# kiudee/bayes-skopt

Hardware: AMD Instinct MI355X
Metric: mcmc_lml_evals_per_s_n2048 (higher is better)
Workload: dtype f64

## Files before the change

bayes-skopt_amd/csrc/bgp_chol.hip:

```cpp
#include "bgp_common.h"
#include "bgp_device.h"

#include "bgp_gemm.h"

#include <cstdlib>
#include <vector>

#ifdef PF_TRACE
__device__ unsigned long long pf_trace[32];
__device__ unsigned long long pf_trace_w[8 * 32];
#define PF_T(i) do { if (threadIdx.x == 0 && blockIdx.x == 0) pf_trace[i] = wall_clock64(); } while (0)
#define PF_TW(i) do { if ((threadIdx.x & 63) == 0 && blockIdx.x == 0) pf_trace_w[(threadIdx.x >> 6) * 32 + (i)] = wall_clock64(); } while (0)
extern "C" int bgp_debug_potrf_trace(unsigned long long* out) {
  return hipMemcpyFromSymbol(out, HIP_SYMBOL(pf_trace), sizeof(pf_trace)) == hipSuccess ? 0 : 1;
}
extern "C" int bgp_debug_potrf_trace_w(unsigned long long* out) {
  return hipMemcpyFromSymbol(out, HIP_SYMBOL(pf_trace_w), sizeof(pf_trace_w)) == hipSuccess ? 0 : 1;
}
#else
#define PF_T(i)
#define PF_TW(i)
#endif
#include "bgp_pf.h"
#include "bgp_mcmc.h"

template <int GEN, int STAT, int FORM>
__global__ void __launch_bounds__(PF_THREADS) potrf_kernel(double* __restrict__ Kbuf, double* __restrict__ Wbuf,
                                                     double* __restrict__ yw, double* __restrict__ accb,
                                                     double* __restrict__ lml, int* __restrict__ status, int n,
                                                     int ld, size_t mstride, int ystride, int nblk, int k, PfGen gen) {
  const int b = blockIdx.x;
  if (!GEN && status[b] != 0) return;
  PfPre nopre;
  nopre.state = 0;
  (void)pf_block<GEN, STAT, FORM, 0>(b, Kbuf, Wbuf, yw, accb, lml, status, n, ld, mstride, ystride, nblk, k, gen, false, nullptr,
                                     PsArgs(), nopre);
}

template <int STAT, int FORM>
__global__ void __launch_bounds__(PF_THREADS) mcmc_small_kernel(McmcArgs a, int h, double* __restrict__ lml, int* __restrict__ status,
                                                               int n, PfGen gen) {
#pragma clang fp contract(off)
  __shared__ double sh_qv[64], sh_pt[64];
  __shared__ double sh_prior;
  __shared__ int sh_acc;
  const int i = blockIdx.x, tid = threadIdx.x, p = a.p;
  const int m = a.movers[(size_t)h * a.Ns + i], pr = a.partners[(size_t)h * a.Ns + i];
  if (tid < p) {
    const double z = a.zz[(size_t)h * a.Ns + i];
    const double s = a.coords[(size_t)m * p + tid], c = a.coords[(size_t)pr * p + tid];
    const double v = c - (c - s) * z;
    sh_qv[tid] = v;
    if (!(v > -INFINITY && v < INFINITY)) {
      a.info[0] = 1u;
      if (v != v) {
        if (a.info[3] == 0u) a.info[3] = (unsigned)h + 1u;
      } else if (a.info[2] == 0u) {
        a.info[2] = (unsigned)h + 1u;
      }
    }
    sh_pt[tid] = mcmc_prior(a.prior_kind[tid], a.prior_par + 5 * tid, v);
  }
  __syncthreads();
  if (tid == 0) {
    double lp = 0.0;
    for (int k = 0; k < p; k++) lp += sh_pt[k];
    sh_prior = lp;
  }
  if (tid < a.hp) a.dh[(size_t)i * a.hp + tid] = a.h_src[tid] >= 0 ? sh_qv[a.h_src[tid]] : a.h_fixed[tid];
  __syncthreads();
  PfPre nopre;
  nopre.state = 0;
  (void)pf_block<1, STAT, FORM, 0>(i, nullptr, nullptr, nullptr, nullptr, lml, status, n, 128, (size_t)0, 0, 1, 0, gen, false, nullptr,
                                   PsArgs(), nopre);
  __syncthreads();
  if (tid == 0) {
    double lp = sh_prior + lml[i];
    if (!(lp > -INFINITY && lp < INFINITY)) lp = -INFINITY;
    const bool acc = a.factors[(size_t)h * a.Ns + i] + lp - a.logp[m] > a.logu[(size_t)h * a.Ns + i];
    if (acc) {
      a.logp[m] = lp;
      a.nacc[m] += 1;
    }
    sh_acc = acc ? 1 : 0;
    a.lps[(size_t)(h >> 1) * a.W + m] = acc ? lp : a.logp[m];
  }
  __syncthreads();
  if (tid < p) {
    const double v = sh_acc ? sh_qv[tid] : a.coords[(size_t)m * p + tid];
    if (sh_acc) a.coords[(size_t)m * p + tid] = v;
    a.chain[((size_t)(h >> 1) * a.W + m) * p + tid] = v;
  }
}

int bgp_launch_mcmc_small(bgp_ctx* ctx, hipStream_t st, const McmcArgs& a, int h) {
  if (a.p > 64 || a.hp > 64) {
    bgp_set_error("bgp_launch_mcmc_small: more than 64 entries per walker");
    return BGP_ERR_INVALID;
  }
  PfGen g;
  g.X = ctx->dXeff;
  g.alpha = ctx->dalpha;
  g.H = ctx->dh;
  g.y = ctx->dy;
  g.d = ctx->d;
  KB_DISPATCH(ctx->ks.stationary, ctx->ks.form,
              hipLaunchKernelGGL((mcmc_small_kernel<S, F>), dim3(a.Ns), dim3(PF_THREADS), 0, st, a, h, ctx->dlml, ctx->dstatus, ctx->n, g));
  BGP_HIP(hipGetLastError());
  return BGP_OK;
}

__global__ void pivot_root_kernel(const double* __restrict__ x, double* __restrict__ s, double* __restrict__ iv, int n) {
  const int i = blockIdx.x * blockDim.x + threadIdx.x;
  if (i >= n) return;
  double a, b;
  pf_pivot_root(x[i], a, b);
  s[i] = a;
  iv[i] = b;
}
extern "C" int bgp_debug_pivot_root(int device, int n, const double* x, double* sqrt_out, double* rsqrt_out) {
  if (n <= 0 || !x || !sqrt_out || !rsqrt_out) {
    bgp_set_error("bgp_debug_pivot_root: bad argument");
    return BGP_ERR_INVALID;
  }
  BGP_HIP(hipSetDevice(device));
  double* d = nullptr;
  BGP_HIP(hipMalloc(&d, (size_t)3 * n * sizeof(double)));
  hipError_t e = hipMemcpy(d, x, (size_t)n * sizeof(double), hipMemcpyHostToDevice);
  if (e == hipSuccess) {
    hipLaunchKernelGGL(pivot_root_kernel, dim3((n + 255) / 256), dim3(256), 0, 0, d, d + n, d + 2 * (size_t)n, n);
    e = hipMemcpy(sqrt_out, d + n, (size_t)n * sizeof(double), hipMemcpyDeviceToHost);
  }
  if (e == hipSuccess) e = hipMemcpy(rsqrt_out, d + 2 * (size_t)n, (size_t)n * sizeof(double), hipMemcpyDeviceToHost);
  (void)hipFree(d);
  BGP_HIP(e);
  return BGP_OK;
}

int bgp_ps_total_tasks(int B, int nblk, int np, int gen);
void bgp_launch_ps(hipStream_t st, const PsArgs& a, int nwg);

extern "C" int bgp_debug_ps_trace(bgp_ctx* c, int* dims, unsigned long long* out, size_t cap) {
  if (!c || !dims) return BGP_ERR_INVALID;
  dims[0] = c->ps_trace_B;
  dims[1] = c->ps_trace_nblk;
  dims[2] = c->ps_trace_total;
  const size_t need = (size_t)c->ps_trace_B * c->ps_trace_nblk * 8 + (size_t)c->ps_trace_total * 8;
  if (!out || !c->ps_trace || need == 0) return BGP_OK;
  if (cap < need) return BGP_ERR_INVALID;
  BGP_HIP(hipSetDevice(c->device));
  BGP_HIP(hipMemcpy(out, c->ps_trace, need * sizeof(unsigned long long), hipMemcpyDeviceToHost));
  return BGP_OK;
}

int bgp_persist_fits(bgp_ctx* c, int B) {
  return B >= 1 && B <= 64 && c->nblk >= 2 && c->nblk <= 255 && c->ncu - B >= std::max(32, B);
}

int bgp_ps_ensure_flags(bgp_ctx* c, int B) {
  const size_t words = ps_flag_words(B, c->nblk);
  if (words > c->cap_psflags) {
    if (c->ps_flags) (void)hipFree(c->ps_flags);
    c->ps_flags = nullptr;
    c->cap_psflags = 0;
    BGP_HIP(hipMalloc(&c->ps_flags, (words + words / 2) * sizeof(unsigned)));
    c->cap_psflags = words + words / 2;
  }
  return BGP_OK;
}

int bgp_launch_cholesky_persist(bgp_ctx* c, int B, int build_gram) {
  const int nblk = c->nblk, ld = c->npad;
  if (!bgp_persist_fits(c, B)) {
    bgp_set_error("bgp_launch_cholesky_persist: B = %d, nblk = %d outside the persistent path's range", B, nblk);
    return BGP_ERR_INVALID;
  }
  const int ncu = c->ncu;
  if (!c->ps_herr) {
    BGP_HIP(hipHostMalloc((void**)&c->ps_herr, sizeof(unsigned), hipHostMallocDefault));
    *c->ps_herr = 0;
  }
  const size_t words = ps_flag_words(B, nblk);
  {
    const int rcf = bgp_ps_ensure_flags(c, B);
    if (rcf) return rcf;
  }
  if (!c->ps_resident) BGP_HIP(hipMemsetAsync(c->ps_flags, 0, words * sizeof(unsigned), c->stream));
  static unsigned long long limit = 0;
  if (!limit) {
    const char* e = getenv("BGP_PS_TIMEOUT_MS");
    limit = 100000ull * (unsigned long long)((e && atoi(e) > 0) ? atoi(e) : 500);
    const char* et = getenv("BGP_PS_TIMEOUT_TICKS");
    if (et && atoll(et) > 0) limit = (unsigned long long)atoll(et);
  }
  PsArgs a;
  a.K = c->dK;
  a.W = c->dW;
  a.yw = c->dyw;
  a.acc = c->dacc;
  a.lml = c->dlml;
  a.status = c->dstatus;
  a.flags = c->ps_flags;
  a.n = c->n;
  a.ld = ld;
  a.nblk = nblk;
  a.B = B;
  a.ystride = ld;
  a.mstride = (size_t)ld * ld;
  {
    static int want = -2;
    if (want == -2) {
      const char* e = getenv("BGP_PS_PAIR");
      want = e ? (atoi(e) != 0 ? 1 : 0) : -1;
    }
    a.Bpad = 8 * ((B + 7) / 8);
    const bool fits = nblk >= 3 && ncu - 2 * a.Bpad >= std::max(32, B);
    a.pair = (fits && (want == 1 || (want == -1 && bgp_pair_auto_rule(nblk, B)))) ? 1 : 0;
    a.nchain = a.pair ? 2 * a.Bpad : B;
    a.psplit = a.pair ? 4 : 1;
    a.dsplit = a.psplit == 4 ? 3 : 1;
    a.total = bgp_ps_total_tasks(B, nblk, a.psplit, 0);
    a.ncrit_stream = 3;
  }
  int tile_wgs = std::min(a.total, ncu - a.nchain);
  {
    const int auto_crit = nblk <= 10 ? ((a.pair || B > 32) ? std::min((a.psplit + 1 + a.dsplit + (a.psplit == 4 ? 4 : 0)) * B, tile_wgs / 2) : 0)
                                     : (a.pair && a.psplit == 4 ? std::min(B == 1 ? 48 : 96, tile_wgs / 2) : 0);
    a.ncrit = auto_crit;
    if (a.ncrit > tile_wgs - 1) a.ncrit = std::max(0, tile_wgs - 1);
  }
  a.gen = 0;
  if (build_gram) {
    static int want = -2;
    if (want == -2) {
      const char* e = getenv("BGP_PS_GEN");
      want = e ? (atoi(e) != 0 ? 1 : 0) : -1;
    }
    const bool can = !a.pair && a.ncrit == 0 && a.total > 0 && c->ks.stationary == BGP_MATERN52 && c->ks.form == BGP_FORM_PRODUCT;
    if (can && (want == 1 || (want == -1 && bgp_ps_gen_auto_rule(nblk, B)))) {
      a.gen = 1;
      a.total = bgp_ps_total_tasks(B, nblk, a.psplit, 1);
    } else {
      const int rck = bgp_launch_kbuild(c, B, 0, 0, 1);
      if (rck) return rck;
    }
  }
  a.d = c->d;
  a.X = c->dXeff;
  a.alpha = c->dalpha;
  a.H = c->dh;
  a.y = c->dy;
  tile_wgs = std::min(a.total, ncu - a.nchain);
  a.spin_limit = limit;
  a.trace = nullptr;
  {
    static int want = -1;
    if (want < 0) {
      const char* e = getenv("BGP_PS_TRACE");
      want = (e && atoi(e) != 0) ? 1 : 0;
    }
    if (want) {
      const size_t need = (size_t)B * nblk * 8 + (size_t)a.total * 8;
      if (need > c->cap_pstrace) {
        if (c->ps_trace) (void)hipFree(c->ps_trace);
        c->ps_trace = nullptr;
        c->cap_pstrace = 0;
        BGP_HIP(hipMalloc(&c->ps_trace, need * sizeof(unsigned long long)));
        c->cap_pstrace = need;
      }
      BGP_HIP(hipMemsetAsync(c->ps_trace, 0, need * sizeof(unsigned long long), c->stream));
      a.trace = c->ps_trace;
      c->ps_trace_B = B;
      c->ps_trace_nblk = nblk;
      c->ps_trace_total = a.total;
    }
  }
  bgp_launch_ps(c->stream, a, a.nchain + tile_wgs);
  if (!c->ps_resident)
    BGP_HIP(hipMemcpyAsync(c->ps_herr, c->ps_flags + PS_ERROR, sizeof(unsigned), hipMemcpyDeviceToHost, c->stream));
  BGP_HIP(hipGetLastError());
  return BGP_OK;
}

void bgp_launch_syrk4(hipStream_t st, int B8, double* dK, const int* dstatus, int ld, size_t mstride, int nblk, int kp,
                      int K, int jstart, int colmode, int B);
void bgp_launch_trsm4(hipStream_t st, int B, double* dK, double* dW, double* dyw, int* dstatus, int ld, size_t mstride,
                      int ystride, int nblk, int k, int augmented);

void bgp_launch_potrf(bgp_ctx* ctx, hipStream_t st, int B, double* dK, double* dW, double* dyw, double* dacc,
                      double* dlml, int* dstatus, int ld, size_t mstride, int ystride, int k) {
  hipLaunchKernelGGL((potrf_kernel<0, 0, 0>), dim3(B), dim3(PF_THREADS), 0, st, dK, dW, dyw, dacc, dlml, dstatus, ctx->n, ld,
                     mstride, ystride, ctx->nblk, k, PfGen());
}

int bgp_launch_lml_small(bgp_ctx* ctx, int off, int B, hipStream_t st) {
  PfGen g;
  g.X = ctx->dXeff;
  g.alpha = ctx->dalpha;
  g.H = ctx->dh + (size_t)off * (ctx->d + 2);
  g.y = ctx->dy;
  g.d = ctx->d;
  bgp_tbegin(ctx, 1, st);
  KB_DISPATCH(ctx->ks.stationary, ctx->ks.form,
              hipLaunchKernelGGL((potrf_kernel<1, S, F>), dim3(B), dim3(PF_THREADS), 0, st, (double*)nullptr,
                                 (double*)nullptr, (double*)nullptr, (double*)nullptr, ctx->dlml + off, ctx->dstatus + off,
                                 ctx->n, 128, (size_t)0, 0, 1, 0, g));
  bgp_tend(ctx, st);
  BGP_HIP(hipGetLastError());
  return BGP_OK;
}

void bgp_launch_syrk4_gen(hipStream_t st, int B8, double* dK, const int* dstatus, int ld, size_t mstride, int nblk, int kp,
                          int K, int jstart, int colmode, int B, const S4Gen& gen, int stationary, int form);

int bgp_launch_cholesky(bgp_ctx* ctx, int B, int augmented) {
  return bgp_launch_cholesky_slice(ctx, 0, B, ctx->stream, augmented);
}

int bgp_launch_cholesky_slice(bgp_ctx* ctx, int off, int B, hipStream_t st, int augmented, int gen) {
  const int nblk = ctx->nblk, npad = ctx->npad;
  const int ld = augmented ? 2 * npad : npad;
  const size_t mstride = (size_t)ld * ld;
  const int ystride = ld;
  const int B8 = 8 * ((B + 7) / 8);
  double* dK = ctx->dK + (size_t)off * mstride;
  double* dW = ctx->dW + (size_t)off * nblk * (128 * 128);
  double* dyw = ctx->dyw + (size_t)off * ystride;
  double* dacc = ctx->dacc + (size_t)off * 4;
  double* dlml = ctx->dlml + off;
  int* dstatus = ctx->dstatus + off;
  if (!augmented) {
    const int P = ctx->panels_auto ? (nblk >= 12 ? 4 : 2) : ctx->panels;
    S4Gen ga{};
    if (gen) {
      const int rcg = bgp_lml_gen_args(ctx, off, &ga);
      if (rcg) return rcg;
      ctx->gen_batches++;
    }
    int k = 0;
// ... 53 lines not shown
```

bayes-skopt_amd/csrc/bgp_pf.h:

```cpp
#pragma once
#include "bgp_common.h"
#include "bgp_device.h"
#include "bgp_gemm.h"

#ifndef PF_T
#define PF_T(i)
#endif
#ifndef PF_TW
#define PF_TW(i)
#endif
#define PF_LD 130
#define PF_MLD 18

template <int C>
static __device__ __forceinline__ double bc16(double v) {
  return __builtin_amdgcn_update_dpp(v, v, 0x150 + C, 0xF, 0xF, false);
}

#define PF_FMAC_BCAST(D, SRC, S1, C)                                                                  \
  asm volatile("v_fmac_f64_dpp %0, %1, %2 row_newbcast:%3 row_mask:0xf bank_mask:0xf" : "+v"(D) : "v"(SRC), "v"(S1), "n"(C))

template <int J, int C>
static __device__ __forceinline__ void micro_cols(double (&a)[16], double (&macc)[16], double naj, double mj) {
  if constexpr (C < 16) {
    PF_FMAC_BCAST(a[C], a[J], naj, C);
    PF_FMAC_BCAST(macc[C], a[J], mj, C);
    micro_cols<J, C + 1>(a, macc, naj, mj);
  }
}

static __device__ __forceinline__ void pf_pivot_root(double x, double& dj, double& inv) {
  const double y0 = __builtin_amdgcn_rsq(x);
  const double g = x * y0, h = 0.5 * y0;
  const double r = fma(-g, h, 0.5);
  const double g1 = fma(g, r, g);
  const double y1 = fma(y0, r, y0);
  const double hy = 0.5 * y1;
  const double d = fma(-g1, g1, x);
  dj = fma(d, hy, g1);
  const double e = fma(-dj, y1, 1.0);
  inv = fma(y1, e, y1);
}

template <int J>
static __device__ __forceinline__ void micro_chol_inv(double (&a)[16], double (&macc)[16], double (&mrow)[16], int lr) {
  if constexpr (J < 16) {
    asm volatile("s_nop 1");
    const double djj = bc16<J>(a[J]);
    double dj, inv;
    pf_pivot_root(djj, dj, inv);
    a[J] = (lr == J) ? dj : a[J] * inv;
    const double naj = -a[J];
    const double mj = (((lr == J) ? 1.0 : 0.0) - macc[J]) * inv;
    mrow[J] = mj;
    if constexpr (J < 15) asm volatile("s_nop 1" ::"v"(a[J]), "v"(naj), "v"(mj));
    micro_cols<J, J + 1>(a, macc, naj, mj);
    micro_chol_inv<J + 1>(a, macc, mrow, lr);
  }
}

static __device__ __forceinline__ void pf_check_diag(const double* __restrict__ s, int blk, int lane, int* fail, int ldt) {
  const int i = blk * 16 + (lane & 15);
  const double v = s[i * ldt + i];
  const unsigned long long m = __ballot(!(v > 0.0 && v < INFINITY)) & 0xffffull;
  if (m != 0 && lane == 0 && *fail == 0) *fail = blk * 16 + __ffsll((long long)m);
}

template <int NEG>
static __device__ __forceinline__ d4 mma_run(d4 acc, const double* __restrict__ pa, const double* __restrict__ pb,
                                             int nt) {
  if (nt <= 0) return acc;
  double a0[4], b0[4];
#pragma unroll
  for (int kk = 0; kk < 4; kk++) {
    a0[kk] = pa[kk * 4];
    b0[kk] = pb[kk * 4];
  }
  for (int t = 0; t < nt; t++) {
    double a1[4], b1[4];
    const int tn = (t + 1 < nt) ? t + 1 : t;
#pragma unroll
    for (int kk = 0; kk < 4; kk++) {
      a1[kk] = pa[tn * 16 + kk * 4];
      b1[kk] = pb[tn * 16 + kk * 4];
    }
#pragma unroll
    for (int kk = 0; kk < 4; kk++) acc = __builtin_amdgcn_mfma_f64_16x16x4f64(NEG ? -a0[kk] : a0[kk], b0[kk], acc, 0, 0, 0);
#pragma unroll
    for (int kk = 0; kk < 4; kk++) {
      a0[kk] = a1[kk];
      b0[kk] = b1[kk];
    }
  }
  return acc;
}

static __device__ __forceinline__ d4 pf_wsum(d4 acc, const double* __restrict__ s, const double* __restrict__ Minv,
                                             const double* __restrict__ xrow, int I, int J, int Kbeg, int Kend,
                                             int lane) {
  const int lr = lane & 15, lk = lane >> 4;
  if (Kbeg == J && Kbeg < Kend) {
#pragma unroll
    for (int kk = 0; kk < 4; kk++) {
      const double av = (J == I - 1 && xrow) ? xrow[lr * PF_MLD + kk * 4 + lk] : s[(I * 16 + lr) * PF_LD + J * 16 + kk * 4 + lk];
      const double bv = Minv[J * 16 * PF_MLD + (kk * 4 + lk) * PF_MLD + lr];
      acc = __builtin_amdgcn_mfma_f64_16x16x4f64(av, bv, acc, 0, 0, 0);
    }
    Kbeg++;
  }
  int Kmid = Kend;
  if (xrow && Kend == I) Kmid = I - 1;
  if (Kmid > Kbeg)
    acc = mma_run<0>(acc, &s[(I * 16 + lr) * PF_LD + Kbeg * 16 + lk], &s[(J * 16 + lr) * PF_LD + Kbeg * 16 + lk],
                     Kmid - Kbeg);
  if (Kmid < Kend && Kmid >= Kbeg) {
#pragma unroll
    for (int kk = 0; kk < 4; kk++) {
      const double av = xrow[lr * PF_MLD + kk * 4 + lk];
      const double bv = s[(J * 16 + lr) * PF_LD + Kmid * 16 + kk * 4 + lk];
      acc = __builtin_amdgcn_mfma_f64_16x16x4f64(av, bv, acc, 0, 0, 0);
    }
  }
  return acc;
}

static __device__ __forceinline__ void pf_wfinish(d4 acc, double* __restrict__ s, const double* __restrict__ Minv,
                                                  double* __restrict__ Wg, int I, int J, int lane) {
  const int lr = lane & 15, lk = lane >> 4;
  d4 wn;
  if (J == I) {
#pragma unroll
    for (int r = 0; r < 4; r++) wn[r] = Minv[I * 16 * PF_MLD + (lk + 4 * r) * PF_MLD + lr];
  } else {
    wn = (d4){0.0, 0.0, 0.0, 0.0};
#pragma unroll
    for (int kk = 0; kk < 4; kk++) {
      const double av = -Minv[I * 16 * PF_MLD + lr * PF_MLD + kk * 4 + lk];
      wn = __builtin_amdgcn_mfma_f64_16x16x4f64(av, acc[kk], wn, 0, 0, 0);
    }
#pragma unroll
    for (int r = 0; r < 4; r++) s[(J * 16 + lr) * PF_LD + I * 16 + lk + 4 * r] = wn[r];
  }
  if (Wg) {
#pragma unroll
    for (int r = 0; r < 4; r++) Wg[(I * 16 + lk + 4 * r) * 128 + J * 16 + lr] = wn[r];
  }
}

#define PF_THREADS 512
struct PfGen {
  const double* X;
  const double* alpha;
  const double* H;
  const double* y;
  int d;
};

template <int STAT, int FORM>
static __device__ __forceinline__ void pf_generate_tile(double* __restrict__ s, double* __restrict__ xs,
                                                        const PfGen& g, const double* __restrict__ h, int n, int tid) {
  const int tx = tid & 15, ty = tid >> 4;
  double acc[4][8];
#pragma unroll
  for (int r = 0; r < 4; r++)
#pragma unroll
    for (int c = 0; c < 8; c++) acc[r][c] = 0.0;
  const int d = g.d;
  for (int k0 = 0; k0 < d; k0 += 16) {
    const int kc = min(16, d - k0);
    __syncthreads();
    for (int idx = tid; idx < kc * 128; idx += PF_THREADS) {
      const int row = idx / kc, kk = idx - row * kc;
      xs[kk * 128 + row] = (row < n) ? g.X[(size_t)row * d + k0 + kk] / exp(h[1 + k0 + kk]) : 0.0;
    }
    __syncthreads();
    for (int kk = 0; kk < kc; kk++) {
      double a[4], bb[8];
#pragma unroll
      for (int r = 0; r < 4; r++) a[r] = xs[kk * 128 + ty + 32 * r];
#pragma unroll
      for (int c = 0; c < 8; c++) bb[c] = xs[kk * 128 + tx + 16 * c];
#pragma unroll
      for (int r = 0; r < 4; r++)
#pragma unroll
        for (int c = 0; c < 8; c++) {
          const double df = a[r] - bb[c];
          acc[r][c] = fma(df, df, acc[r][c]);
        }
    }
  }
  {
#pragma clang fp contract(off)
  const double cst = exp(h[0]), s2 = exp(h[d + 1]);
#pragma unroll
  for (int r = 0; r < 4; r++) {
    const int gi = ty + 32 * r;
#pragma unroll
    for (int c = 0; c < 8; c++) {
      const int gj = tx + 16 * c;
      double v;
      if (gi >= n || gj >= n) {
        v = (gi == gj) ? 1.0 : 0.0;
      } else if (gi == gj) {
        const double base = (FORM == BGP_FORM_PRODUCT) ? cst * 1.0 : cst + 1.0;
        v = (base + s2) + g.alpha[gi];
      } else {
        const double sv = kb_stationary<STAT>(acc[r][c]);
        v = (FORM == BGP_FORM_PRODUCT) ? cst * sv : cst + sv;
      }
      s[gi * PF_LD + gj] = v;
    }
  }
}
}

struct PfLds {
  double* s;
  double* Minv;
  double* xrow;
  double* ylds;
  double* zpart;
  double* red;
  int* fail;
};
#define PF_LDS_BYTES ((128 * PF_LD + 8 * 16 * PF_MLD + 2 * 16 * PF_MLD + 128 + 4 * 128 + 16) * 8 + 16)
static __device__ __forceinline__ char* pf_lds_raw() {
  __shared__ __attribute__((aligned(1024))) char raw[PF_LDS_BYTES];
  return raw;
}
static __device__ __forceinline__ PfLds pf_lds() {
  double* const base = reinterpret_cast<double*>(pf_lds_raw());
  PfLds l;
  l.s = base;
  l.Minv = l.s + 128 * PF_LD;
  l.xrow = l.Minv + 8 * 16 * PF_MLD;
  l.ylds = l.xrow + 2 * 16 * PF_MLD;
  l.zpart = l.ylds + 128;
  l.red = l.zpart + 4 * 128;
  l.fail = reinterpret_cast<int*>(l.red + 16);
  return l;
}

struct PfPre {
  double af[32];
  int state;
};
static __device__ __forceinline__ void pf_pre_issue(const PsArgs& a, int b, int J, int w, int lr, int lk, PfPre& pre) {
  const int I = J + 1, ld = a.ld;
  const double* const Ab = a.K + (size_t)b * a.mstride + (size_t)I * 128 * ld + (size_t)J * 128;
  pf_afrag_issue(Ab + (size_t)(16 * w + lr) * ld, lk, pre.af);
  pre.state = 2;
}

template <int GEN, int STAT, int FORM, int PRE>
static __device__ __forceinline__ int pf_block(int b, double* __restrict__ Kbuf, double* __restrict__ Wbuf,
                                               double* __restrict__ yw, double* __restrict__ accb,
                                               double* __restrict__ lml, int* __restrict__ status, int n, int ld,
                                               size_t mstride, int ystride, int nblk, int k, const PfGen& gen,
                                               bool inlds, unsigned* wrow, const PsArgs& pa, PfPre& pre) {
  const PfLds lds = pf_lds();
  double* const s = lds.s;
  double* const Minv = lds.Minv;
  double* const xrow0 = lds.xrow;
  double* const ylds = lds.ylds;
  double* const zpart = lds.zpart;
  double* const red = lds.red;
  int& fail_lds = *lds.fail;
  int tid_ = threadIdx.x;
  asm volatile("" : "+v"(tid_));
  const int tid = tid_, lane = tid & 63, w = tid >> 6;
  const int lr = lane & 15, lk = lane >> 4;
  double* T = Kbuf + (size_t)b * mstride + (size_t)(k * 128) * ld + k * 128;
  double* yk = yw + (size_t)b * ystride + k * 128;
  PF_T(0);

  if (GEN) {
    if (tid == 0) status[b] = 0;
    pf_generate_tile<STAT, FORM>(s, Minv, gen, gen.H + (size_t)b * (gen.d + 2), n, tid);
  } else if (!inlds) {
    const int seg = tid & 63, rbase = tid >> 6;
    d2 v[16];
#pragma unroll
    for (int u = 0; u < 16; u++) {
      const int row = rbase + 8 * u;
      v[u] = (2 * seg <= row + 15) ? *reinterpret_cast<const d2*>(T + (size_t)row * ld + seg * 2) : (d2){0.0, 0.0};
    }
#pragma unroll
    for (int u = 0; u < 16; u++) {
      const int row = rbase + 8 * u;
      *reinterpret_cast<d2*>(&s[row * PF_LD + seg * 2]) = v[u];
    }
  }
  if (tid < 128 && !inlds) ylds[tid] = GEN ? gen.y[tid] : yk[tid];
  double ld_prev = 0.0, zz_prev = 0.0;
  if (tid == 0) {
    fail_lds = 0;
    if (PRE) lds.fail[1] = 0;
    if (k > 0) {
      ld_prev = accb[b * 4 + 0];
      zz_prev = accb[b * 4 + 1];
    }
  }
  __syncthreads();
  PF_T(1);

  double* Wg = GEN ? nullptr : Wbuf + ((size_t)b * nblk + k) * (128 * 128);
  int failed = 0;
  d4 xpend = (d4){0.0, 0.0, 0.0, 0.0};
  d4 w7 = (d4){0.0, 0.0, 0.0, 0.0};
  const int u6 = (w < 4) ? w - 1 : w - 2;
  unsigned pre_fs = 0, pre_fd = 0;
  int pre_seen = (PRE && k + 1 < nblk) ? 0 : 1;
#pragma unroll 1
  for (int sb = 0; sb < 8; sb++) {
    PF_TW(2 * sb);
    if (PRE && w == 4 && lane == 0 && !pre_seen) {
      const bool gen0 = k == 0 && pa.gen;
      const unsigned want_s = gen0 ? 1u : (unsigned)pa.psplit, want_d = gen0 ? 1u : (unsigned)pa.dsplit;
      if ((k == 0 && !pa.gen) || (sb > 0 && pre_fs >= want_s && pre_fd >= want_d)) {
        if (k > 0 || pa.gen) ps_acquire();
        lds.fail[1] = 1;
        pre_seen = 1;
      } else if (gen0) {
        const unsigned* const g1 = pa.flags + PS_GEN(pa.B, nblk) + ((size_t)b * nblk + 1) * nblk;
        pre_fs = ps_ld(g1 + 0);
        pre_fd = ps_ld(g1 + 1);
      } else {
        pre_fd = ps_ld(pa.flags + PS_HDR + (size_t)pa.B * nblk + (size_t)b * nblk + (k + 1));
        pre_fs = ps_ld(pa.flags + PS_HDR + (size_t)pa.B * nblk * (2 + nblk) + (size_t)b * nblk + (k + 1));
      }
    }
    if (w == 4 && sb > 0) pf_check_diag(s, sb - 1, lane, lds.fail, PF_LD);
    if (w == 0) {
      if (sb > 1) {
#pragma unroll
        for (int r = 0; r < 4; r++) s[((sb - 1) * 16 + lr) * PF_LD + (sb - 2) * 16 + lk + 4 * r] = xpend[r];
      }
      d4 dg;
#pragma unroll
      for (int r = 0; r < 4; r++) dg[r] = s[(sb * 16 + lk + 4 * r) * PF_LD + sb * 16 + lr];
      if (sb > 0) {
        d4 xt = (d4){0.0, 0.0, 0.0, 0.0};
#pragma unroll
        for (int kk = 0; kk < 4; kk++) {
          const double av = Minv[(sb - 1) * 16 * PF_MLD + lr * PF_MLD + kk * 4 + lk];
          const double bv = s[(sb * 16 + lr) * PF_LD + (sb - 1) * 16 + kk * 4 + lk];
          xt = __builtin_amdgcn_mfma_f64_16x16x4f64(av, bv, xt, 0, 0, 0);
        }
#pragma unroll
        for (int kk = 0; kk < 4; kk++) dg = __builtin_amdgcn_mfma_f64_16x16x4f64(-xt[kk], xt[kk], dg, 0, 0, 0);
        xpend = xt;
#pragma unroll
        for (int r = 0; r < 4; r++) xrow0[(sb & 1) * 16 * PF_MLD + lr * PF_MLD + lk + 4 * r] = xt[r];
      }
#pragma unroll
      for (int r = 0; r < 4; r++) s[(sb * 16 + lk + 4 * r) * PF_LD + sb * 16 + lr] = dg[r];
      double a[16], mrow[16], macc[16];
#pragma unroll
      for (int c = 0; c < 16; c++) {
        a[c] = s[(sb * 16 + lr) * PF_LD + sb * 16 + c];
        macc[c] = 0.0;
      }
#ifdef PF_TRACE
      asm volatile("s_nop 0" ::"v"(a[0]), "v"(a[15]));
#endif
      PF_T(3 + sb * 3);
      micro_chol_inv<0>(a, macc, mrow, lr);
#ifdef PF_TRACE
      asm volatile("s_nop 0" ::"v"(a[15]), "v"(mrow[15]), "v"(mrow[14]));
#endif
      PF_T(4 + sb * 3);
      if (lane < 16) {
#pragma unroll
        for (int j = 0; j < 16; j++) Minv[sb * 16 * PF_MLD + j * PF_MLD + lr] = mrow[j];
#pragma unroll
        for (int c = 0; c < 16; c++) s[(sb * 16 + lr) * PF_LD + sb * 16 + c] = (c <= lr) ? a[c] : 0.0;
      }
    } else if (sb > 0 && w != 4) {
      const int p = sb - 1;
      d4 xt = (d4){0.0, 0.0, 0.0, 0.0};
      if (p + 2 < 8) {
#pragma unroll
        for (int kk = 0; kk < 4; kk++) {
          const double av = Minv[p * 16 * PF_MLD + lr * PF_MLD + kk * 4 + lk];
          const double bv = s[((p + 1) * 16 + lr) * PF_LD + p * 16 + kk * 4 + lk];
          xt = __builtin_amdgcn_mfma_f64_16x16x4f64(av, bv, xt, 0, 0, 0);
        }
      }
      for (int I = p + 2 + u6; I < 8; I += 6) {
        d4 xi = (d4){0.0, 0.0, 0.0, 0.0};
#pragma unroll
        for (int kk = 0; kk < 4; kk++) {
          const double av = Minv[p * 16 * PF_MLD + lr * PF_MLD + kk * 4 + lk];
          const double bv = s[(I * 16 + lr) * PF_LD + p * 16 + kk * 4 + lk];
          xi = __builtin_amdgcn_mfma_f64_16x16x4f64(av, bv, xi, 0, 0, 0);
        }
        d4 acc;
#pragma unroll
        for (int r = 0; r < 4; r++) acc[r] = s[(I * 16 + lk + 4 * r) * PF_LD + (p + 1) * 16 + lr];
        if (p > 0)
          acc = mma_run<1>(acc, &s[(I * 16 + lr) * PF_LD + (p - 1) * 16 + lk],
                           &s[((p + 1) * 16 + lr) * PF_LD + (p - 1) * 16 + lk], 1);
#pragma unroll
        for (int kk = 0; kk < 4; kk++) acc = __builtin_amdgcn_mfma_f64_16x16x4f64(-xi[kk], xt[kk], acc, 0, 0, 0);
#pragma unroll
        for (int r = 0; r < 4; r++) s[(I * 16 + lk + 4 * r) * PF_LD + (p + 1) * 16 + lr] = acc[r];
#pragma unroll
        for (int r = 0; r < 4; r++) s[(I * 16 + lr) * PF_LD + p * 16 + lk + 4 * r] = xi[r];
        if (p > 0 || I == p + 2) {
#pragma unroll
          for (int r = 0; r < 4; r++) acc[r] = s[(I * 16 + lk + 4 * r) * PF_LD + (p + 2) * 16 + lr];
          acc = mma_run<1>(acc, &s[(I * 16 + lr) * PF_LD + lk], &s[((p + 2) * 16 + lr) * PF_LD + lk], p);
          if (I == p + 2) {
#pragma unroll
            for (int kk = 0; kk < 4; kk++) acc = __builtin_amdgcn_mfma_f64_16x16x4f64(-xi[kk], xi[kk], acc, 0, 0, 0);
          }
#pragma unroll
          for (int r = 0; r < 4; r++) s[(I * 16 + lk + 4 * r) * PF_LD + (p + 2) * 16 + lr] = acc[r];
        }
      }
      for (int J = 5 - u6; J <= p; J += 6) {
        d4 acc = (d4){0.0, 0.0, 0.0, 0.0};
        if (J < p) acc = pf_wsum(acc, s, Minv, xrow0 + (p & 1) * 16 * PF_MLD, p, J, J, p, lane);
        pf_wfinish(acc, s, Minv, Wg, p, J, lane);
      }
      if (!GEN && sb >= 2 && sb <= 6) {
        const int R = sb - 2, ut = u6 * 64 + lane;
        const int rr = ut / 24, c0 = ut - 24 * rr, row = R * 16 + rr;
        for (int seg = c0; seg < 8 * R + 8; seg += 24) {
          if (2 * seg <= row)
            *reinterpret_cast<d2*>(T + (size_t)row * ld + seg * 2) = *reinterpret_cast<const d2*>(&s[row * PF_LD + seg * 2]);
        }
      }
      if (sb == 7) w7 = pf_wsum(w7, s, Minv, nullptr, 7, u6, u6, 6, lane);
      if (wrow) asm volatile("s_waitcnt vmcnt(0)" ::: "memory");
    }
    PF_TW(2 * sb + 1);
    __syncthreads();
    PF_T(2 + sb * 3);
    failed = fail_lds;
    if (failed) break;
    if (wrow && w == 4 && lane == 0 && sb >= 1) {
      ps_release();
      ps_st(wrow, (unsigned)sb);
    }
  }
  if (!failed && w == 4) pf_check_diag(s, 7, lane, lds.fail, PF_LD);
  if (failed) {
    if (tid == 0) {
      status[b] = k * 128 + failed;
      lml[b] = -INFINITY;
    }
    return failed;
  }
  PF_T(26);
  if (!GEN) {
    const int seg = tid & 63, rbase = tid >> 6;
#pragma unroll
    for (int i = 10; i < 16; i++) {
      const int row = rbase + 8 * i;
      if (2 * seg <= row && !(row >= 112 && seg >= 48 && seg < 56))
        *reinterpret_cast<d2*>(T + (size_t)row * ld + seg * 2) = *reinterpret_cast<const d2*>(&s[row * PF_LD + seg * 2]);
    }
  }
  if (w == 0) {
    if (!GEN) {
#pragma unroll
      for (int r = 0; r < 4; r++) T[(size_t)(7 * 16 + lr) * ld + 6 * 16 + lk + 4 * r] = xpend[r];
    }
    d4 acc = (d4){0.0, 0.0, 0.0, 0.0};
    acc = pf_wsum(acc, s, Minv, xrow0 + 16 * PF_MLD, 7, 6, 6, 7, lane);
    pf_wfinish(acc, s, Minv, Wg, 7, 6, lane);
    pf_wfinish(acc, s, Minv, Wg, 7, 7, lane);
  } else if (w != 4) {
    w7 = pf_wsum(w7, s, Minv, xrow0 + 16 * PF_MLD, 7, u6, 6, 7, lane);
    pf_wfinish(w7, s, Minv, Wg, 7, u6, lane);
  }
  double ldv = (tid < 128) ? log(s[tid * PF_LD + tid]) : 0.0;
  for (int o = 32; o > 0; o >>= 1) ldv += __shfl_xor(ldv, o);
  if (lane == 0) red[w] = ldv;
  __syncthreads();
  failed = fail_lds;
  if (failed) {
    if (tid == 0) {
      status[b] = k * 128 + failed;
      lml[b] = -INFINITY;
    }
    return failed;
  }
  PF_T(27);
  {
    const int row = tid & 127, h = tid >> 7, Ib = row >> 4, ri = row & 15;
    double z0 = 0.0, z1 = 0.0;
    for (int j = h; j < 16 * Ib; j += 8) {
      z0 = fma(s[j * PF_LD + row], ylds[j], z0);
      z1 = fma(s[(j + 4) * PF_LD + row], ylds[j + 4], z1);
    }
    double zs = z0 + z1;
    for (int jj = h; jj <= ri; jj += 4) zs = fma(Minv[Ib * 16 * PF_MLD + ri * PF_MLD + jj], ylds[16 * Ib + jj], zs);
    zpart[h * 128 + row] = zs;
  }
  __syncthreads();
  double zv = 0.0;
  if (tid < 128) {
    zv = (zpart[tid] + zpart[128 + tid]) + (zpart[256 + tid] + zpart[384 + tid]);
    if (!GEN) yk[tid] = zv;
    zpart[tid] = zv;
  }
  double zz = zv * zv;
  for (int o = 32; o > 0; o >>= 1) zz += __shfl_xor(zz, o);
  if (lane == 0) red[8 + w] = zz;
  __syncthreads();
  if (tid == 0) {
    double ldt = red[0] + red[1];
    double zzt = red[8] + red[9];
    ldt += ld_prev;
    zzt += zz_prev;
    if (!GEN) {
      accb[b * 4 + 0] = ldt;
      accb[b * 4 + 1] = zzt;
    }
    if (k == nblk - 1) {
#pragma clang fp contract(off)
      double v = -0.5 * zzt - ldt - 0.5 * (double)n * 1.8378770664093453;
      if (!(v > -INFINITY && v < INFINITY)) {
        v = -INFINITY;
        status[b] = n + 1;
      }
      lml[b] = v;
    }
  }
  PF_T(28);
  __syncthreads();
  return 0;
}

template <int NT>
static __device__ __forceinline__ void pf_diag_update(d4 (&dt)[5], const double* __restrict__ s, const int (&offa)[5],
                                                      const int (&offb)[5]) {
  double a0[NT], b0[NT];
#pragma unroll
  for (int u = 0; u < NT; u++) {
    a0[u] = s[offa[u]];
    b0[u] = s[offb[u]];
  }
#pragma unroll 2
  for (int t = 0; t < 32; t++) {
    double a1[NT], b1[NT];
    const int tn = (t + 1 < 32) ? t + 1 : t;
#pragma unroll
    for (int u = 0; u < NT; u++) {
      a1[u] = s[offa[u] + 4 * tn];
      b1[u] = s[offb[u] + 4 * tn];
    }
#pragma unroll
    for (int u = 0; u < NT; u++) dt[u] = __builtin_amdgcn_mfma_f64_16x16x4f64(a0[u], b0[u], dt[u], 0, 0, 1);
#pragma unroll
    for (int u = 0; u < NT; u++) {
      a0[u] = a1[u];
      b0[u] = b1[u];
    }
  }
}

static __device__ __forceinline__ int pf_chain_next(const PsArgs& a, int b, int J, int* ok_lds, unsigned long long* tr, PfPre& pre) {
  const PfLds lds = pf_lds();
  double* const s = lds.s;
  const double* const Minv = lds.Minv;
  double* const ylds = lds.ylds;
  const double* const zl = lds.zpart;
  int tid_ = threadIdx.x;
  asm volatile("" : "+v"(tid_));
  const int tid = tid_, lane = tid & 63;
  const int w = __builtin_amdgcn_readfirstlane(tid >> 6);
  const int lr = lane & 15, lk = lane >> 4;
  const int I = J + 1, ld = a.ld, nblk = a.nblk;
  unsigned* const flags = a.flags;
  unsigned* const err = flags + PS_ERROR;
  double* const Mb = a.K + (size_t)b * a.mstride;
  double* const Ab = Mb + (size_t)I * 128 * ld + (size_t)J * 128;
  const double* const Db = Mb + (size_t)I * 128 * ld + (size_t)I * 128;
  const bool early = pre.state == 2;
  if ((J > 0 || a.gen) && !early) {
    if (tid == 0) {
      const unsigned* const diagrdy = flags + PS_HDR + (size_t)a.B * nblk + (size_t)b * nblk;
      const unsigned* const subrdy = flags + PS_HDR + (size_t)a.B * nblk * (2 + nblk) + (size_t)b * nblk;
      const unsigned* const g1 = flags + PS_GEN(a.B, nblk) + ((size_t)b * nblk + 1) * nblk;
      const bool ok = J > 0 ? ps_wait_ge2(subrdy + I, (unsigned)a.psplit, diagrdy + I, (unsigned)a.dsplit, err, a.spin_limit)
                            : ps_wait_ge2(g1 + 0, 1u, g1 + 1, 1u, err, a.spin_limit);
      ps_acquire();
      *ok_lds = ok ? 1 : 0;
    }
    __syncthreads();
    if (!*ok_lds) return -1;
  }
  if (tr && tid == 0) tr[J * 8 + 2] = wall_clock64();
  if (!early) pf_pre_issue(a, b, J, w, lr, lk, pre);
  pre.state = 0;
  double (&af)[32] = pre.af;
  double yv[4];
  {
    const double* const yi = a.yw + (size_t)b * a.ystride + I * 128;
#pragma unroll
    for (int r = 0; r < 4; r++) yv[r] = yi[16 * w + lk + 4 * r];
  }
  pf_afrag_transpose(af);
// ... 539 lines not shown
```

Baseline: 17040.

## Overlap status check with tile load and split first panel load across waves

The status-based early exit moves from the kernel entry into pf_block, so the skip flag load overlaps with the tile and y loads instead of serializing ahead of them. The tile load is restructured so wave 0 loads only the first 16-row panel while the other waves load the remaining rows. The block-wide barrier is removed on this path, which appears intended to let wave 0 start the first diagonal factorization without waiting for the whole tile. Correctness now depends on later synchronization before other waves read the rows they did not load, and skipped blocks still pay for the tile loads. It also adds per-block trace timestamps under PF_TRACE.

```diff
diff --git a/bayes-skopt_amd/csrc/bgp_chol.hip b/bayes-skopt_amd/csrc/bgp_chol.hip
--- a/bayes-skopt_amd/csrc/bgp_chol.hip
+++ b/bayes-skopt_amd/csrc/bgp_chol.hip
@@ -9,10 +9,18 @@
 #ifdef PF_TRACE
 __device__ unsigned long long pf_trace[32];
 __device__ unsigned long long pf_trace_w[8 * 32];
-#define PF_T(i) do { if (threadIdx.x == 0 && blockIdx.x == 0) pf_trace[i] = wall_clock64(); } while (0)
+__device__ unsigned long long pf_trace_b[2 * 1024];
+#define PF_T(i)                                                                                                          \
+  do {                                                                                                                   \
+    if (threadIdx.x == 0 && blockIdx.x == 0) pf_trace[i] = wall_clock64();                                               \
+    if (threadIdx.x == 0 && ((i) == 0 || (i) == 28) && blockIdx.x < 1024) pf_trace_b[2 * blockIdx.x + ((i) == 28)] = wall_clock64(); \
+  } while (0)
 #define PF_TW(i) do { if ((threadIdx.x & 63) == 0 && blockIdx.x == 0) pf_trace_w[(threadIdx.x >> 6) * 32 + (i)] = wall_clock64(); } while (0)
 extern "C" int bgp_debug_potrf_trace(unsigned long long* out) {
   return hipMemcpyFromSymbol(out, HIP_SYMBOL(pf_trace), sizeof(pf_trace)) == hipSuccess ? 0 : 1;
+}
+extern "C" int bgp_debug_potrf_trace_b(unsigned long long* out) {
+  return hipMemcpyFromSymbol(out, HIP_SYMBOL(pf_trace_b), sizeof(pf_trace_b)) == hipSuccess ? 0 : 1;
 }
 extern "C" int bgp_debug_potrf_trace_w(unsigned long long* out) {
   return hipMemcpyFromSymbol(out, HIP_SYMBOL(pf_trace_w), sizeof(pf_trace_w)) == hipSuccess ? 0 : 1;
@@ -30,11 +38,10 @@
                                                      double* __restrict__ lml, int* __restrict__ status, int n,
                                                      int ld, size_t mstride, int ystride, int nblk, int k, PfGen gen) {
   const int b = blockIdx.x;
-  if (!GEN && status[b] != 0) return;
   PfPre nopre;
   nopre.state = 0;
   (void)pf_block<GEN, STAT, FORM, 0>(b, Kbuf, Wbuf, yw, accb, lml, status, n, ld, mstride, ystride, nblk, k, gen, false, nullptr,
-                                     PsArgs(), nopre);
+                                     PsArgs(), nopre, GEN ? nullptr : status);
 }
 
 template <int STAT, int FORM>
diff --git a/bayes-skopt_amd/csrc/bgp_pf.h b/bayes-skopt_amd/csrc/bgp_pf.h
--- a/bayes-skopt_amd/csrc/bgp_pf.h
+++ b/bayes-skopt_amd/csrc/bgp_pf.h
@@ -257,7 +257,8 @@
                                                double* __restrict__ yw, double* __restrict__ accb,
                                                double* __restrict__ lml, int* __restrict__ status, int n, int ld,
                                                size_t mstride, int ystride, int nblk, int k, const PfGen& gen,
-                                               bool inlds, unsigned* wrow, const PsArgs& pa, PfPre& pre) {
+                                               bool inlds, unsigned* wrow, const PsArgs& pa, PfPre& pre,
+                                               const int* __restrict__ skip = nullptr) {
   const PfLds lds = pf_lds();
   double* const s = lds.s;
   double* const Minv = lds.Minv;
@@ -273,10 +274,45 @@
   double* T = Kbuf + (size_t)b * mstride + (size_t)(k * 128) * ld + k * 128;
   double* yk = yw + (size_t)b * ystride + k * 128;
   PF_T(0);
+  const bool split = !GEN && !inlds && !PRE;
+  int skipped = 0;
+  if (skip) {
+    int bv = b;
+    asm volatile("" : "+v"(bv));
+    skipped = skip[bv];
+  }
+  double yv = 0.0;
+  if (!GEN && !inlds && tid < 128) yv = yk[tid];
+  double ld_prev = 0.0, zz_prev = 0.0;
+  if (tid == 0 && k > 0) {
+    ld_prev = accb[b * 4 + 0];
+    zz_prev = accb[b * 4 + 1];
+  }
 
   if (GEN) {
     if (tid == 0) status[b] = 0;
     pf_generate_tile<STAT, FORM>(s, Minv, gen, gen.H + (size_t)b * (gen.d + 2), n, tid);
+  } else if (split) {
+    if (w == 0) {
+      const int seg = lane & 7, row = lane >> 3;
+      const d2 v0 = *reinterpret_cast<const d2*>(T + (size_t)row * ld + seg * 2);
+      const d2 v1 = *reinterpret_cast<const d2*>(T + (size_t)(row + 8) * ld + seg * 2);
+      *reinterpret_cast<d2*>(&s[row * PF_LD + seg * 2]) = v0;
+      *reinterpret_cast<d2*>(&s[(row + 8) * PF_LD + seg * 2]) = v1;
+    } else {
+      const int seg = lane, rbase = 16 + (w - 1);
+      d2 v[16];
+#pragma unroll
+      for (int u = 0; u < 16; u++) {
+        const int row = rbase + 7 * u;
+        v[u] = (2 * seg <= row + 15) ? *reinterpret_cast<const d2*>(T + (size_t)row * ld + seg * 2) : (d2){0.0, 0.0};
+      }
+#pragma unroll
+      for (int u = 0; u < 16; u++) {
+        const int row = rbase + 7 * u;
+        *reinterpret_cast<d2*>(&s[row * PF_LD + seg * 2]) = v[u];
+      }
+    }
   } else if (!inlds) {
     const int seg = tid & 63, rbase = tid >> 6;
     d2 v[16];
@@ -291,17 +327,13 @@
       *reinterpret_cast<d2*>(&s[row * PF_LD + seg * 2]) = v[u];
     }
   }
-  if (tid < 128 && !inlds) ylds[tid] = GEN ? gen.y[tid] : yk[tid];
-  double ld_prev = 0.0, zz_prev = 0.0;
+  if (skip && __builtin_amdgcn_readfirstlane(skipped) != 0) return 0;
+  if (tid < 128 && !inlds) ylds[tid] = GEN ? gen.y[tid] : yv;
   if (tid == 0) {
     fail_lds = 0;
     if (PRE) lds.fail[1] = 0;
-    if (k > 0) {
-      ld_prev = accb[b * 4 + 0];
-      zz_prev = accb[b * 4 + 1];
-    }
-  }
-  __syncthreads();
+  }
+  if (!split) __syncthreads();
   PF_T(1);
 
   double* Wg = GEN ? nullptr : Wbuf + ((size_t)b * nblk + k) * (128 * 128);
```

After: 17080 (median of 5 runs). Within noise of the previous version (+0.2%).
